# cvg/glue-factory

Measured on AMD Instinct MI355X. Metric: image-pairs/sec (train step) SP+LightGlue N=2048 d=256 L=9, higher is better.
Workload: dtype bf16; 1 GPU; configs[1]: SuperPoint + LightGlue train step -- frozen SuperPoint-open forward on 2x32 synthetic 1024x1024 images resident in HBM (view1 = view0 warped by a sampled homography, SURVEY 8(d)(P); first block and the 64-channel 3x3 blocks as fused HIP kernels, library convolutions + fused HIP tails for the 128/256-channel blocks), homography ground truth (gf_gt_nn), LightGlue fwd + loss + bwd + fused; pairs_per_gpu=32, global_batch=32, keypoints=2048, descriptor_dim=256, layers=9, parallelism=dp1

## Files before the change

### glue-factory_amd/csrc/gemm_st.hip

```cpp
#include <type_traits>
#include "gf_common.h"
#include "gf_amd.h"

namespace {

typedef unsigned int u32x4 __attribute__((ext_vector_type(4)));
typedef unsigned int u32x2 __attribute__((ext_vector_type(2)));
typedef __attribute__((address_space(3))) void gs_lds_void;
typedef const __attribute__((address_space(1))) void gs_glb_void;

constexpr int GS_TILE = 32768;
#ifndef GS_NSTAGE_
#define GS_NSTAGE_ 3
#endif
#ifndef GS_WGS
#define GS_WGS 256
#endif
constexpr int GS_NSTAGE = GS_NSTAGE_, GS_PD = GS_NSTAGE - 1;

struct GsParams {
    const bf16_t* x0; const bf16_t* x1; const bf16_t* w; const float* bias; const bf16_t* res; const bf16_t* res2; bf16_t* y;
    const float* cs;
    int M, N;
    int64_t ld0, ld1, ldw, ldr, ldr2, ldy;
};

template <int OFF> __device__ __forceinline__ u32x4 gs_rd128(unsigned a) {
    u32x4 v;
    asm volatile("ds_read_b128 %0, %1 offset:%2" : "=v"(v) : "v"(a), "n"(OFF) : "memory");
    return v;
}
template <int N> __device__ __forceinline__ void gs_wait_lgkm() { asm volatile("s_waitcnt lgkmcnt(%0)" ::"n"(N) : "memory"); }
template <int N> __device__ __forceinline__ void gs_wait_vm() { asm volatile("s_waitcnt vmcnt(%0)" ::"n"(N) : "memory"); }
template <typename V> __device__ __forceinline__ void gs_tie(V& v) { asm volatile("" : "+v"(v)); }
__device__ __forceinline__ u32x4 gs_ld128(const void* p) {
    u32x4 v;
    asm volatile("global_load_dwordx4 %0, %1, off" : "=v"(v) : "v"(p) : "memory");
    return v;
}
__device__ __forceinline__ void gs_st128(void* p, u32x4 v) {
    asm volatile("global_store_dwordx4 %0, %1, off\n\ts_nop 2" ::"v"(p), "v"(v) : "memory");
}
__device__ __forceinline__ void gs_swap(unsigned& a, unsigned& b) {
    const auto r = __builtin_amdgcn_permlane32_swap(a, b, false, false);
    a = r[0]; b = r[1];
}

template <int KF, bool TWO, int RES, bool ROT>
__global__ __launch_bounds__(512, 2) void gemm_st_kernel(GsParams p) {
    extern __shared__ __attribute__((aligned(1024))) char smem[];
    constexpr int K = 16 * KF, ROWB = 2 * K, CPR = ROWB / 16;
    constexpr int TR = GS_TILE / ROWB, NRB = TR / 32;
    constexpr int NR = RES * 2 * NRB + (ROT ? 4 * NRB : 0), NS = 2 * NRB;
    const unsigned lds0 = (unsigned)(size_t)smem;
    const int lane = threadIdx.x & 63, wave = __builtin_amdgcn_readfirstlane(threadIdx.x >> 6);
    const int l31 = lane & 31, hi = lane >> 5;
    const int ch0 = blockIdx.y * 256 + wave * 32;
    const int ntile = p.M / TR;
    const int T = (ntile - (int)blockIdx.x + (int)gridDim.x - 1) / (int)gridDim.x;
    if (T <= 0) return;

    bf16x8 wf[KF];
#pragma unroll
    for (int s = 0; s < KF; ++s) wf[s] = *reinterpret_cast<const bf16x8*>(p.w + (int64_t)(ch0 + l31) * p.ldw + 16 * s + 8 * hi);
    float bias16[16];
#pragma unroll
    for (int r = 0; r < 16; ++r) bias16[r] = p.bias ? p.bias[ch0 + crow(r, hi)] : 0.f;
    gs_wait_vm<0>();

    auto issue = [&](int i, int stage) {
        const int ti = (int)blockIdx.x + min(i, T - 1) * (int)gridDim.x;
#pragma unroll
        for (int j = 0; j < 4; ++j) {
            const int piece = 4 * wave + j;
            const int lin = 64 * piece + lane;
            const int row = lin / CPR, c = (lin % CPR) ^ (row & 15);
            const int64_t grow = (int64_t)ti * TR + row;
            const bf16_t* src = (TWO && c >= CPR / 2) ? p.x1 + grow * p.ld1 + (c - CPR / 2) * 8 : p.x0 + grow * p.ld0 + c * 8;
            __builtin_amdgcn_global_load_lds((gs_glb_void*)src, (gs_lds_void*)(smem + stage * GS_TILE + piece * 1024), 16, 0, 0);
        }
    };
#pragma unroll
    for (int t = 0; t < GS_PD; ++t) issue(t, t);

    unsigned a0[8];
#pragma unroll
    for (int sl = 0; sl < 8; ++sl) a0[sl] = lds0 + (unsigned)(l31 * ROWB + (((2 * sl + hi) ^ (l31 & 15)) << 4));
    const int64_t ycol = ch0 + 8 * hi;

    for (int i = 0; i < T; ++i) {
        const int stage = i % GS_NSTAGE;
        const int64_t row0 = ((int64_t)blockIdx.x + (int64_t)i * gridDim.x) * TR;
        constexpr int PER = NR + 4 + NS;
        if (i >= GS_PD) gs_wait_vm<NS + (GS_PD - 1) * PER>();
        else if (i == 0) gs_wait_vm<(GS_PD - 1) * 4>();
        else if (i == 1) gs_wait_vm<(GS_PD > 1 ? (GS_PD - 2) * 4 + PER : 0)>();
        else gs_wait_vm<(GS_PD > 2 ? (GS_PD - 3) * 4 + 2 * PER : 0)>();
        __builtin_amdgcn_s_barrier();
        __builtin_amdgcn_sched_barrier(0);
        u32x4 rr[NRB][2], rq[NRB][2];
        if (RES >= 1) {
#pragma unroll
            for (int rb = 0; rb < NRB; ++rb)
#pragma unroll
                for (int j = 0; j < 2; ++j) rr[rb][j] = gs_ld128(p.res + (row0 + 32 * rb + l31) * p.ldr + ycol + 16 * j);
        }
        if (RES == 2) {
#pragma unroll
            for (int rb = 0; rb < NRB; ++rb)
#pragma unroll
                for (int j = 0; j < 2; ++j) rq[rb][j] = gs_ld128(p.res2 + (row0 + 32 * rb + l31) * p.ldr2 + ycol + 16 * j);
        }
        u32x4 cc[NRB][4];
        if (ROT) {
#pragma unroll
            for (int rb = 0; rb < NRB; ++rb)
#pragma unroll
                for (int g = 0; g < 4; ++g)
                    cc[rb][g] = gs_ld128(p.cs + (row0 + 32 * rb + l31) * 64 + (wave & 1) * 32 + 8 * g + 4 * hi);
        }
        issue(i + GS_PD, (i + GS_PD) % GS_NSTAGE);
        unsigned a[8];
#pragma unroll
        for (int sl = 0; sl < 8; ++sl) a[sl] = a0[sl] + stage * GS_TILE;

        f32x16 acc[NRB];
        u32x4 xa[4], xb[4];
        auto rd = [&](u32x4 (&dst)[4], auto RB, auto G) {
            constexpr int rb = decltype(RB)::value, g = decltype(G)::value;
#pragma unroll
            for (int q = 0; q < 4; ++q) dst[q] = gs_rd128<rb * 32 * ROWB + ((4 * g) / 8) * 256>(a[(4 * g + q) & 7]);
        };
        auto mma = [&](u32x4 (&src)[4], auto RB, auto G) {
            constexpr int rb = decltype(RB)::value, g = decltype(G)::value;
#pragma unroll
            for (int q = 0; q < 4; ++q) {
                gs_tie(src[q]);
                acc[rb] = __builtin_amdgcn_mfma_f32_32x32x16_bf16(wf[4 * g + q], __builtin_bit_cast(bf16x8, src[q]), acc[rb], 0, 0, 0);
            }
        };
        auto block = [&](auto RB) {
            constexpr int rb = decltype(RB)::value, NG = KF / 4;
#pragma unroll
            for (int r = 0; r < 16; ++r) acc[rb][r] = bias16[r];
            rd(xa, RB, std::integral_constant<int, 0>{});
            rd(xb, RB, std::integral_constant<int, 1>{});
            auto step = [&](u32x4 (&buf)[4], auto G) {
                constexpr int g = decltype(G)::value;
                if constexpr (g < NG) {
                    if constexpr (g == NG - 1) gs_wait_lgkm<0>(); else gs_wait_lgkm<4>();
                    mma(buf, RB, G);
                    if constexpr (g + 2 < NG) rd(buf, RB, std::integral_constant<int, g + 2>{});
                }
            };
            step(xa, std::integral_constant<int, 0>{}); step(xb, std::integral_constant<int, 1>{});
            step(xa, std::integral_constant<int, 2>{}); step(xb, std::integral_constant<int, 3>{});
            step(xa, std::integral_constant<int, 4>{}); step(xb, std::integral_constant<int, 5>{});
            step(xa, std::integral_constant<int, 6>{}); step(xb, std::integral_constant<int, 7>{});
        };
        block(std::integral_constant<int, 0>{});
        if constexpr (NRB > 1) block(std::integral_constant<int, 1>{});
        if (RES || ROT) gs_wait_vm<4>();
#pragma unroll
        for (int rb = 0; rb < NRB; ++rb) {
            bf16_t* yp = p.y + (row0 + 32 * rb + l31) * p.ldy + ycol;
#pragma unroll
            for (int j = 0; j < 2; ++j) {
                float v[2][4];
#pragma unroll
                for (int e = 0; e < 4; ++e) { v[0][e] = acc[rb][8 * j + e]; v[1][e] = acc[rb][8 * j + 4 + e]; }
                if (ROT) {
#pragma unroll
                    for (int t = 0; t < 2; ++t) {
                        gs_tie(cc[rb][2 * j + t]);
                        const f32x4 c = __builtin_bit_cast(f32x4, cc[rb][2 * j + t]);
                        const float o0 = v[t][0] * c[0] - v[t][1] * c[1], o1 = v[t][1] * c[0] + v[t][0] * c[1];
                        const float o2 = v[t][2] * c[2] - v[t][3] * c[3], o3 = v[t][3] * c[2] + v[t][2] * c[3];
                        v[t][0] = o0; v[t][1] = o1; v[t][2] = o2; v[t][3] = o3;
                    }
                }
                auto add_res = [&](u32x4& src) {
                    gs_tie(src);
                    unsigned a0_ = src[0], a1_ = src[1], b0_ = src[2], b1_ = src[3];
                    gs_swap(a0_, b0_);
                    gs_swap(a1_, b1_);
                    const bf16x4 r0 = __builtin_bit_cast(bf16x4, u32x2{a0_, a1_}), r1 = __builtin_bit_cast(bf16x4, u32x2{b0_, b1_});
#pragma unroll
                    for (int e = 0; e < 4; ++e) { v[0][e] += (float)r0[e]; v[1][e] += (float)r1[e]; }
                };
                if (RES >= 1) add_res(rr[rb][j]);
                if (RES == 2) add_res(rq[rb][j]);
                const bf16x4 o0 = {(bf16_t)v[0][0], (bf16_t)v[0][1], (bf16_t)v[0][2], (bf16_t)v[0][3]};
                const bf16x4 o1 = {(bf16_t)v[1][0], (bf16_t)v[1][1], (bf16_t)v[1][2], (bf16_t)v[1][3]};
                const u32x2 p0 = __builtin_bit_cast(u32x2, o0), p1 = __builtin_bit_cast(u32x2, o1);
                unsigned q0 = p0[0], q1 = p0[1], q2 = p1[0], q3 = p1[1];
                gs_swap(q0, q2);
                gs_swap(q1, q3);
                gs_st128(yp + 16 * j, u32x4{q0, q1, q2, q3});
            }
        }
    }
    gs_wait_vm<0>();
}

template <int KF, bool TWO, int RES, bool ROT = false>
int gs_launch(const GsParams& p, hipStream_t st) {
    constexpr int TR = GS_TILE / (32 * KF);
    const size_t lds = (size_t)GS_NSTAGE * GS_TILE;
    hipError_t e = hipFuncSetAttribute(reinterpret_cast<const void*>(gemm_st_kernel<KF, TWO, RES, ROT>),
                                       hipFuncAttributeMaxDynamicSharedMemorySize, (int)lds);
    if (e != hipSuccess) return (int)e;
    const int ntile = p.M / TR, ncg = p.N / 256;
    int gx = GS_WGS / ncg;
    if (gx < 1) gx = 1;
    if (gx > ntile) gx = ntile;
    gemm_st_kernel<KF, TWO, RES, ROT><<<dim3(gx, ncg), dim3(512), lds, st>>>(p);
    return (int)hipGetLastError();
}

}

int gf_gemm_stream_try(const void* x0, const void* x1, const void* w, const float* bias, const void* res, void* y,
                       const float* cs, int rot_n, int M, int N, int K0, int K1, int64_t ld0, int64_t ld1, int64_t ldw,
                       int64_t ldr, int64_t ldy, hipStream_t st, const void* res2, int64_t ldr2) {
    const int K = K0 + K1;
    if ((K != 256 && K != 512) || N % 256 || M % 64 || (K1 && K1 != K0)) return GF_ERR_UNSUPPORTED;
    if (cs && (rot_n % 256 || rot_n <= 0 || rot_n > N || res || K1)) return GF_ERR_UNSUPPORTED;
    if (res2 && (!res || cs)) return GF_ERR_UNSUPPORTED;
    GsParams p;
    p.x0 = static_cast<const bf16_t*>(x0); p.x1 = static_cast<const bf16_t*>(x1); p.w = static_cast<const bf16_t*>(w);
    p.bias = bias; p.res = static_cast<const bf16_t*>(res); p.res2 = static_cast<const bf16_t*>(res2);
    p.y = static_cast<bf16_t*>(y); p.cs = cs;
    p.M = M; p.N = N; p.ld0 = ld0; p.ld1 = ld1; p.ldw = ldw; p.ldr = ldr; p.ldr2 = ldr2; p.ldy = ldy;
    if (cs) {
        p.N = rot_n;
        if (int e = K == 256 ? gs_launch<16, false, 0, true>(p, st) : gs_launch<32, false, 0, true>(p, st)) return e;
        if (N == rot_n) return 0;
        p.N = N - rot_n; p.w += (int64_t)rot_n * ldw; p.y += rot_n; p.cs = nullptr;
        if (p.bias) p.bias += rot_n;
        return K == 256 ? gs_launch<16, false, 0>(p, st) : gs_launch<32, false, 0>(p, st);
    }
    if (res2) return K1 ? (K == 256 ? gs_launch<16, true, 2>(p, st) : gs_launch<32, true, 2>(p, st))
                        : (K == 256 ? gs_launch<16, false, 2>(p, st) : gs_launch<32, false, 2>(p, st));
#define GS_GO(KF) (K1 ? (res ? gs_launch<KF, true, 1>(p, st) : gs_launch<KF, true, 0>(p, st)) \
                      : (res ? gs_launch<KF, false, 1>(p, st) : gs_launch<KF, false, 0>(p, st)))
    return K == 256 ? GS_GO(16) : GS_GO(32);
#undef GS_GO
}
```

Measured before the change: 532.3 image-pairs/s.

## Stage rotary cos/sin table through LDS pipeline in streaming GEMM

With default settings (GS_ABL=0), the rotary cos/sin table for each tile is now fetched asynchronously into LDS alongside the activation tile using global_load_lds. The epilogue reads it from LDS instead of issuing direct per-thread global loads. This folds the table traffic into the multi-stage prefetch pipeline so the epilogue no longer waits on it, and the vmcnt accounting is updated to match. Each stage's LDS footprint grows, which may cut occupancy. Ablation flags also add experiments that skip stores, use a fake identity rotation or remap stores, but these are off by default.

Measured after the change: 533.0 image-pairs/s, median of 6. No clear change (+0.1%).

```diff
diff --git a/glue-factory_amd/csrc/gemm_st.hip b/glue-factory_amd/csrc/gemm_st.hip
--- a/glue-factory_amd/csrc/gemm_st.hip
+++ b/glue-factory_amd/csrc/gemm_st.hip
@@ -17,6 +17,9 @@
 #define GS_WGS 256
 #endif
 constexpr int GS_NSTAGE = GS_NSTAGE_, GS_PD = GS_NSTAGE - 1;
+#ifndef GS_ABL
+#define GS_ABL 0
+#endif
 
 struct GsParams {
     const bf16_t* x0; const bf16_t* x1; const bf16_t* w; const float* bias; const bf16_t* res; const bf16_t* res2; bf16_t* y;
@@ -39,6 +42,7 @@
     return v;
 }
 __device__ __forceinline__ void gs_st128(void* p, u32x4 v) {
+    if (GS_ABL & 8) return;
     asm volatile("global_store_dwordx4 %0, %1, off\n\ts_nop 2" ::"v"(p), "v"(v) : "memory");
 }
 __device__ __forceinline__ void gs_swap(unsigned& a, unsigned& b) {
@@ -51,7 +55,9 @@
     extern __shared__ __attribute__((aligned(1024))) char smem[];
     constexpr int K = 16 * KF, ROWB = 2 * K, CPR = ROWB / 16;
     constexpr int TR = GS_TILE / ROWB, NRB = TR / 32;
-    constexpr int NR = RES * 2 * NRB + (ROT ? 4 * NRB : 0), NS = 2 * NRB;
+    constexpr bool TBL = ROT && !(GS_ABL & 4);
+    constexpr int STAGE = GS_TILE + (TBL ? TR * 256 : 0);
+    constexpr int NR = RES * 2 * NRB, PC = 4 + (TBL ? NRB : 0), NS = (GS_ABL & 8) ? 0 : 2 * NRB;
     const unsigned lds0 = (unsigned)(size_t)smem;
     const int lane = threadIdx.x & 63, wave = __builtin_amdgcn_readfirstlane(threadIdx.x >> 6);
     const int l31 = lane & 31, hi = lane >> 5;
@@ -66,9 +72,10 @@
     float bias16[16];
 #pragma unroll
     for (int r = 0; r < 16; ++r) bias16[r] = p.bias ? p.bias[ch0 + crow(r, hi)] : 0.f;
-    gs_wait_vm<0>();
+    if (!(GS_ABL & 1)) gs_wait_vm<0>();
 
     auto issue = [&](int i, int stage) {
+        if ((GS_ABL & 2) && i >= T) return;
         const int ti = (int)blockIdx.x + min(i, T - 1) * (int)gridDim.x;
 #pragma unroll
         for (int j = 0; j < 4; ++j) {
@@ -77,7 +84,16 @@
             const int row = lin / CPR, c = (lin % CPR) ^ (row & 15);
             const int64_t grow = (int64_t)ti * TR + row;
             const bf16_t* src = (TWO && c >= CPR / 2) ? p.x1 + grow * p.ld1 + (c - CPR / 2) * 8 : p.x0 + grow * p.ld0 + c * 8;
-            __builtin_amdgcn_global_load_lds((gs_glb_void*)src, (gs_lds_void*)(smem + stage * GS_TILE + piece * 1024), 16, 0, 0);
+            __builtin_amdgcn_global_load_lds((gs_glb_void*)src, (gs_lds_void*)(smem + stage * STAGE + piece * 1024), 16, 0, 0);
+        }
+        if (TBL) {
+#pragma unroll
+            for (int j = 0; j < NRB; ++j) {
+                const int piece = NRB * wave + j;
+                const int row = 4 * piece + (lane >> 4), c = (lane & 15) ^ (row & 15);
+                const float* src = p.cs + ((int64_t)ti * TR + row) * 64 + c * 4;
+                __builtin_amdgcn_global_load_lds((gs_glb_void*)src, (gs_lds_void*)(smem + stage * STAGE + GS_TILE + piece * 1024), 16, 0, 0);
+            }
         }
     };
 #pragma unroll
@@ -86,16 +102,19 @@
     unsigned a0[8];
 #pragma unroll
     for (int sl = 0; sl < 8; ++sl) a0[sl] = lds0 + (unsigned)(l31 * ROWB + (((2 * sl + hi) ^ (l31 & 15)) << 4));
+    unsigned c0[4];
+#pragma unroll
+    for (int g = 0; g < 4; ++g) c0[g] = lds0 + (unsigned)(GS_TILE + l31 * 256 + ((((wave & 1) * 8 + 2 * g + hi) ^ (l31 & 15)) << 4));
     const int64_t ycol = ch0 + 8 * hi;
 
     for (int i = 0; i < T; ++i) {
         const int stage = i % GS_NSTAGE;
         const int64_t row0 = ((int64_t)blockIdx.x + (int64_t)i * gridDim.x) * TR;
-        constexpr int PER = NR + 4 + NS;
+        constexpr int PER = NR + PC + NS;
         if (i >= GS_PD) gs_wait_vm<NS + (GS_PD - 1) * PER>();
-        else if (i == 0) gs_wait_vm<(GS_PD - 1) * 4>();
-        else if (i == 1) gs_wait_vm<(GS_PD > 1 ? (GS_PD - 2) * 4 + PER : 0)>();
-        else gs_wait_vm<(GS_PD > 2 ? (GS_PD - 3) * 4 + 2 * PER : 0)>();
+        else if (i == 0) gs_wait_vm<(GS_PD - 1) * PC>();
+        else if (i == 1) gs_wait_vm<(GS_PD > 1 ? (GS_PD - 2) * PC + PER : 0)>();
+        else gs_wait_vm<(GS_PD > 2 ? (GS_PD - 3) * PC + 2 * PER : 0)>();
         __builtin_amdgcn_s_barrier();
         __builtin_amdgcn_sched_barrier(0);
         u32x4 rr[NRB][2], rq[NRB][2];
@@ -111,20 +130,13 @@
 #pragma unroll
                 for (int j = 0; j < 2; ++j) rq[rb][j] = gs_ld128(p.res2 + (row0 + 32 * rb + l31) * p.ldr2 + ycol + 16 * j);
         }
-        u32x4 cc[NRB][4];
-        if (ROT) {
-#pragma unroll
-            for (int rb = 0; rb < NRB; ++rb)
-#pragma unroll
-                for (int g = 0; g < 4; ++g)
-                    cc[rb][g] = gs_ld128(p.cs + (row0 + 32 * rb + l31) * 64 + (wave & 1) * 32 + 8 * g + 4 * hi);
-        }
         issue(i + GS_PD, (i + GS_PD) % GS_NSTAGE);
         unsigned a[8];
 #pragma unroll
-        for (int sl = 0; sl < 8; ++sl) a[sl] = a0[sl] + stage * GS_TILE;
+        for (int sl = 0; sl < 8; ++sl) a[sl] = a0[sl] + stage * STAGE;
 
         f32x16 acc[NRB];
+        u32x4 cc[NRB][4];
         u32x4 xa[4], xb[4];
         auto rd = [&](u32x4 (&dst)[4], auto RB, auto G) {
             constexpr int rb = decltype(RB)::value, g = decltype(G)::value;
@@ -143,6 +155,13 @@
             constexpr int rb = decltype(RB)::value, NG = KF / 4;
 #pragma unroll
             for (int r = 0; r < 16; ++r) acc[rb][r] = bias16[r];
+            if (TBL) {
+#pragma unroll
+                for (int g = 0; g < 4; ++g) cc[rb][g] = gs_rd128<rb * 32 * 256>(c0[g] + stage * STAGE);
+            } else if (ROT) {
+#pragma unroll
+                for (int g = 0; g < 4; ++g) cc[rb][g] = __builtin_bit_cast(u32x4, f32x4{1.f, 0.f, 1.f, 0.f});
+            }
             rd(xa, RB, std::integral_constant<int, 0>{});
             rd(xb, RB, std::integral_constant<int, 1>{});
             auto step = [&](u32x4 (&buf)[4], auto G) {
@@ -160,10 +179,11 @@
         };
         block(std::integral_constant<int, 0>{});
         if constexpr (NRB > 1) block(std::integral_constant<int, 1>{});
-        if (RES || ROT) gs_wait_vm<4>();
+        if (RES) gs_wait_vm<PC>();
 #pragma unroll
         for (int rb = 0; rb < NRB; ++rb) {
             bf16_t* yp = p.y + (row0 + 32 * rb + l31) * p.ldy + ycol;
+            if (GS_ABL & 16) yp = p.y + (row0 + 32 * rb + 2 * wave + hi) * p.ldy + blockIdx.y * 256 + 8 * l31;
 #pragma unroll
             for (int j = 0; j < 2; ++j) {
                 float v[2][4];
@@ -196,7 +216,7 @@
                 unsigned q0 = p0[0], q1 = p0[1], q2 = p1[0], q3 = p1[1];
                 gs_swap(q0, q2);
                 gs_swap(q1, q3);
-                gs_st128(yp + 16 * j, u32x4{q0, q1, q2, q3});
+                gs_st128((GS_ABL & 16) ? yp + 16 * j * p.ldy : yp + 16 * j, u32x4{q0, q1, q2, q3});
             }
         }
     }
@@ -206,7 +226,7 @@
 template <int KF, bool TWO, int RES, bool ROT = false>
 int gs_launch(const GsParams& p, hipStream_t st) {
     constexpr int TR = GS_TILE / (32 * KF);
-    const size_t lds = (size_t)GS_NSTAGE * GS_TILE;
+    const size_t lds = (size_t)GS_NSTAGE * (GS_TILE + (ROT && !(GS_ABL & 4) ? TR * 256 : 0));
     hipError_t e = hipFuncSetAttribute(reinterpret_cast<const void*>(gemm_st_kernel<KF, TWO, RES, ROT>),
                                        hipFuncAttributeMaxDynamicSharedMemorySize, (int)lds);
     if (e != hipSuccess) return (int)e;
```
